# nilsbore/gp_compressor

Measured on AMD Instinct MI355X. Metric: patches/sec (compress+predict), higher is better.
Workload: dtype f64; 1 GPU; C2 room scan: 8192 patches x 256 pts per GPU, RBF + Gaussian noise, dense Cholesky fit + predictive mean on the 20x20 grid (m=400); patches_per_gpu=8192, points_per_patch=256, grid_points=400, parallelism=1 GPU, kernel=dense_mfma_w1

## Files before the change

gp_compressor_amd/csrc/dense_mfma_w1.hip:

```cpp
#include <cstdio>
#include <cstdlib>
#include <type_traits>

#include "gpc_device.h"
#include "dense_internal.h"
#include "mfma_tile.h"

#define W1_NPAD_MAX 512
#define W1_C 4
#define W1_NDT 10
#define W1_NT_OF(npad) ((npad) / 16)
#define W1_TRI_OF(npad) (W1_NT_OF(npad) * (W1_NT_OF(npad) + 1) / 2)
#define W1_TILE(i, j) (((size_t)(i) * (size_t)((i) + 1) / 2 + (size_t)(j)) * MF_IMG)


struct W1Params {
    DenseArgs a;
    double c_exp;
    double pivot_tol;
    double cs, noise_u, sfp, a_out;
    double* ws;
    double* linvt;
    int export_factor;
    unsigned long long* stamps;
};
#define W1_NPH 12
#ifdef W1_STAMPS
#define W1_STAMP(ph)                                                                                                 \
    do {                                                                                                             \
        __builtin_amdgcn_sched_barrier(0);                                                                           \
        const unsigned long long t_now_ = __builtin_amdgcn_s_memtime();                                              \
        st_acc_[ph] += t_now_ - t_prev_;                                                                             \
        t_prev_ = t_now_;                                                                                            \
        __builtin_amdgcn_sched_barrier(0);                                                                           \
    } while (0)
#else
#define W1_STAMP(ph) do { } while (0)
#endif

#define W1_LDS_SYNC()                                                                                                \
    do {                                                                                                             \
        __builtin_amdgcn_fence(__ATOMIC_SEQ_CST, "wavefront");                                                       \
        __builtin_amdgcn_wave_barrier();                                                                             \
    } while (0)

template <int A, int B, typename F>
__device__ static __forceinline__ void w1_static_for(F&& f)
{
    if constexpr (A < B) {
        f(std::integral_constant<int, A>{});
        w1_static_for<A + 1, B>(f);
    }
}
__host__ __device__ constexpr int w1_stream_col(int q)
{
    int kk = 0;
    while ((kk + 1) * (kk + 2) / 2 <= q) ++kk;
    return kk;
}
#define W1_BW 20

__device__ static __forceinline__ d4 w1_mfma4_neg(d4 a, d4 b, d4 acc)
{
#pragma unroll
    for (int s = 0; s < 4; ++s) acc = __builtin_amdgcn_mfma_f64_16x16x4f64(a[s], b[s], acc, 0, 0, 1);
    return acc;
}
__device__ static __forceinline__ d4 w1_trsm(d4 lv, d4 src)
{
    const d4 z4 = d4{0.0, 0.0, 0.0, 0.0};
    d4 D = __builtin_amdgcn_mfma_f64_16x16x4f64(lv[0], src[0], z4, 0, 0, 0);
    D = __builtin_amdgcn_mfma_f64_16x16x4f64(lv[1], src[1], D, 0, 0, 0);
    D = __builtin_amdgcn_mfma_f64_16x16x4f64(lv[2], src[2], D, 0, 0, 0);
    return __builtin_amdgcn_mfma_f64_16x16x4f64(lv[3], src[3], D, 0, 0, 0);
}

template <int MODE, int CNT, bool DIAG>
__device__ static __forceinline__ void w1_gram_row(d4 (&v)[W1_C], const double* px0, const double* px1, const double* T, double sf, bool scale_sf,
                                                   double cexp, double noise, bool dbl, int n, int r, int c0, int lr, int lg)
{
    const int pi = MF_TS * r + lr;
    const double xi0 = px0[pi], xi1 = px1[pi];
#pragma unroll
    for (int t = 0; t < CNT; ++t) {
#pragma unroll
        for (int q = 0; q < 4; ++q) {
            const int pj = MF_TS * (c0 + t) + lg + 4 * q;
            const double d0 = xi0 - px0[pj], d1 = xi1 - px1[pj];
            const double sq = __builtin_fma(d0, d0, d1 * d1);
            v[t][q] = MODE == 0 ? gpc_exp_neg(cexp * sq, T) : gpc_expm_poly<MODE == 1 ? 7 : 5>(sq);
        }
    }
    if (scale_sf) {
#pragma unroll
        for (int t = 0; t < CNT; ++t)
#pragma unroll
            for (int q = 0; q < 4; ++q) v[t][q] *= sf;
    }
    if constexpr (DIAG) {
#pragma unroll
        for (int q = 0; q < 4; ++q) {
            double d = v[CNT - 1][q] + noise;
            if (dbl) d += noise;
            v[CNT - 1][q] = (lr == lg + 4 * q) ? d : v[CNT - 1][q];
        }
    }
    if (MF_TS * (r + 1) > n || MF_TS * (c0 + CNT) > n) {
#pragma unroll
        for (int t = 0; t < CNT; ++t) {
#pragma unroll
            for (int q = 0; q < 4; ++q) {
                const int pj = MF_TS * (c0 + t) + lg + 4 * q;
                if (pi >= n || pj >= n) v[t][q] = (pi == pj) ? 1.0 : 0.0;
            }
        }
    }
}

template <int W1_NPAD>
__global__ __launch_bounds__(64, 2) void dense_w1_kernel(W1Params g)
{
    constexpr int W1_NT = W1_NT_OF(W1_NPAD), W1_TRI = W1_TRI_OF(W1_NPAD);
    __shared__ __attribute__((aligned(16))) double T[GPC_EXP_TABLE_SIZE];
    __shared__ __attribute__((aligned(16))) double px0[W1_NPAD], px1[W1_NPAD], zv[W1_NPAD];
    __shared__ __attribute__((aligned(16))) double rsbuf[32], wsc[32];
    __shared__ __attribute__((aligned(16))) double LinvC[W1_C * MF_IMG];

    const DenseArgs& A = g.a;
    int lane = threadIdx.x;
    int lr = lane & 15, lg = lane >> 4;
#define W1_FRESH_LANE()                                                                                              \
    do {                                                                                                             \
        lane = mf_opaque(lane);                                                                                      \
        lr = lane & 15;                                                                                              \
        lg = lane >> 4;                                                                                              \
    } while (0)
    const int m = A.m;
    const double sf = A.prm.sigmaf_sq, cexp = g.c_exp;
    const bool dbl = A.prm.ref_double_noise != 0;
    const int patch = blockIdx.x;
    double* Lt = g.ws + (size_t)patch * W1_TRI * MF_IMG;
    double* LinvTg = g.linvt + (size_t)patch * W1_NT * MF_IMG;

    gpc_exp_table_init(T);
    {
        const int o = __builtin_amdgcn_readfirstlane(A.off[patch]);
        const int n = __builtin_amdgcn_readfirstlane(A.off[patch + 1]) - o;
        double* fs = A.f_star + (size_t)patch * m;
        __syncthreads();
        if (n <= 0 || n > W1_NPAD) {
            for (int p = lane; p < m; p += 64) fs[p] = (n == 0) ? 0.0 : __builtin_nan("");
            if (lane == 0 && A.status) A.status[patch] = (n == 0) ? GPC_STATUS_OK : GPC_STATUS_NAN;
            return;
        }
        const int nt = __builtin_amdgcn_readfirstlane((n + MF_TS - 1) / MF_TS);
#ifdef W1_STAMPS
        unsigned long long st_acc_[W1_NPH] = {};
        unsigned long long t_prev_ = __builtin_amdgcn_s_memtime();
#endif

        const double xo0 = A.x0[o], xo1 = A.x1[o];
        double qr0[W1_NPAD / 64], qr1[W1_NPAD / 64];
        double mn0 = xo0, mx0 = xo0, mn1 = xo1, mx1 = xo1;
#pragma unroll
        for (int u = 0; u < W1_NPAD / 64; ++u) {
            const int i = lane + 64 * u;
            const bool live = i < n;
            qr0[u] = live ? A.x0[o + i] : xo0;
            qr1[u] = live ? A.x1[o + i] : xo1;
            mn0 = __builtin_fmin(mn0, qr0[u]); mx0 = __builtin_fmax(mx0, qr0[u]);
            mn1 = __builtin_fmin(mn1, qr1[u]); mx1 = __builtin_fmax(mx1, qr1[u]);
            zv[i] = live ? A.y[o + i] : 0.0;
        }
#pragma unroll
        for (int o_ = 32; o_ > 0; o_ >>= 1) {
            mn0 = __builtin_fmin(mn0, __shfl_xor(mn0, o_, 64)); mx0 = __builtin_fmax(mx0, __shfl_xor(mx0, o_, 64));
            mn1 = __builtin_fmin(mn1, __shfl_xor(mn1, o_, 64)); mx1 = __builtin_fmax(mx1, __shfl_xor(mx1, o_, 64));
        }
        int mode_g, mode_p;
        {
            const bool nan_box = !((mx0 - mn0) + (mx1 - mn1) < __builtin_inf());
            const double rx = mx0 - mn0, ry = mx1 - mn1;
            const double tg = nan_box ? __builtin_inf() : -cexp * __builtin_fma(rx, rx, ry * ry);
            const double hb = 0.5 * A.grid_res;
            const double bx = hb + __builtin_fmax(__builtin_fabs(mn0), __builtin_fabs(mx0));
            const double by = hb + __builtin_fmax(__builtin_fabs(mn1), __builtin_fabs(mx1));
            const double bq = __builtin_fmax(bx, by);
            const double tp = nan_box ? __builtin_inf() : -cexp * (bq * bq);
            mode_g = __builtin_amdgcn_readfirstlane(tg <= GPC_EXP_TINY_MAX ? 2 : tg <= GPC_EXP_SMALL_MAX ? 1 : 0);
            mode_p = __builtin_amdgcn_readfirstlane(tp <= GPC_EXP_TINY_MAX ? 2 : tp <= GPC_EXP_SMALL_MAX ? 1 : 0);
            if (mode_g == 0) mode_p = 0;
        }
        const bool scaled = mode_g > 0;
        {
            const double cs = scaled ? g.cs : 1.0;
            const double co0 = scaled ? xo0 : 0.0, co1 = scaled ? xo1 : 0.0;
#pragma unroll
            for (int u = 0; u < W1_NPAD / 64; ++u) {
                const int i = lane + 64 * u;
                const bool live = i < n;
                px0[i] = live ? cs * (qr0[u] - co0) : 0.0;
                px1[i] = live ? cs * (qr1[u] - co1) : 0.0;
            }
        }
        const bool scale_sf = g.export_factor != 0;
        const double noise_u = g.noise_u, ptol = g.pivot_tol;
        W1_LDS_SYNC();
#define W1_GRAM_ROW(v, CNT, DIAG, r, c0)                                                                              \
    do {                                                                                                             \
        if (mode_g == 2) w1_gram_row<2, CNT, DIAG>(v, px0, px1, T, sf, scale_sf, cexp, noise_u, dbl, n, r, c0, lr, lg);   \
        else if (mode_g == 1) w1_gram_row<1, CNT, DIAG>(v, px0, px1, T, sf, scale_sf, cexp, noise_u, dbl, n, r, c0, lr, lg); \
        else w1_gram_row<0, CNT, DIAG>(v, px0, px1, T, sf, scale_sf, cexp, noise_u, dbl, n, r, c0, lr, lg);            \
    } while (0)

        auto bw_step = [&](auto P, const d4 img, d4& pa) __attribute__((always_inline)) {
            constexpr int q = decltype(P)::value;
            constexpr int kk = w1_stream_col(q), t = q - kk * (kk + 1) / 2;
            if (kk < nt) {
                const int k = nt - 1 - kk;
                if constexpr (t < kk) {
                    const double a_ = zv[MF_TS * (k + 1 + t) + lr];
                    pa += img * a_;
                } else {
                    d4 ub = d4{0.0, 0.0, 0.0, 0.0};
                    if constexpr (kk > 0) {
                        const double tot = mf_row_reduce4(pa, lr);
                        if ((lr & 3) == 0) wsc[lg + 4 * (lr >> 2)] = tot;
                        W1_LDS_SYNC();
                        if (lr == 0) {
#pragma unroll
                            for (int q4 = 0; q4 < 4; ++q4) ub[q4] = zv[MF_TS * k + lg + 4 * q4] - wsc[lg + 4 * q4];
                        }
                    } else {
                        if (lr == 0) {
#pragma unroll
                            for (int q4 = 0; q4 < 4; ++q4) ub[q4] = zv[MF_TS * k + lg + 4 * q4];
                        }
                    }
                    const d4 al = w1_trsm(img, ub);
                    W1_LDS_SYNC();
                    if (lr == 0) {
#pragma unroll
                        for (int r = 0; r < 4; ++r) zv[MF_TS * k + lg + 4 * r] = al[r];
                    }
                    W1_LDS_SYNC();
                    pa = d4{0.0, 0.0, 0.0, 0.0};
                }
            }
        };
        bool bad = false;
        W1_STAMP(0);
#define W1_BLOCK_ROW(bi, kb, nb)                                                                                     \
    do {                                                                                                             \
        if ((bi) < (nb)) {                                                                                           \
            d4 gv[W1_C];                                                                                             \
            W1_GRAM_ROW(gv, (bi) + 1, true, (kb) + (bi), (kb));                                                      \
            _Pragma("unroll") for (int bc = 0; bc <= (bi); ++bc) tacc[(bi) * ((bi) + 1) / 2 + bc] = gv[bc];           \
        } else {                                                                                                     \
            _Pragma("unroll") for (int bc = 0; bc <= (bi); ++bc) tacc[(bi) * ((bi) + 1) / 2 + bc] = d4{0.0, 0.0, 0.0, 0.0}; \
        }                                                                                                            \
    } while (0)
#define W1_BLOCK_INIT(kb, nb)                                                                                        \
    do {                                                                                                             \
        _Pragma("unroll") for (int i = 0; i < W1_C; ++i) part[i] = 0.0;                                              \
                                             \
        __builtin_amdgcn_sched_barrier(0);                                                                           \
        W1_BLOCK_ROW(3, kb, nb);                                                                                     \
        __builtin_amdgcn_sched_barrier(0);                                                                           \
        W1_BLOCK_ROW(2, kb, nb);                                                                                     \
        __builtin_amdgcn_sched_barrier(0);                                                                           \
        W1_BLOCK_ROW(1, kb, nb);                                                                                     \
        __builtin_amdgcn_sched_barrier(0);                                                                           \
        W1_BLOCK_ROW(0, kb, nb);                                                                                     \
        __builtin_amdgcn_sched_barrier(0);                                                                           \
    } while (0)
        W1_STAMP(1);
        for (int k = 0;; k += W1_C) {
            const int nc = min(W1_C, nt - k);
            const int kl = k - 1;
            const bool last_step = k + W1_C >= nt;
            (void)last_step;
            W1_FRESH_LANE();
            const double* rrow[W1_C];
#pragma unroll
            for (int i = 0; i < W1_C; ++i) rrow[i] = Lt + W1_TILE(k + min(i, nc - 1), 0);
            d4 tacc[W1_NDT];
            double part[W1_C];
            d4 op[2][W1_C];
#pragma unroll
            for (int i = 0; i < W1_C; ++i) op[0][i] = op[1][i] = d4{0.0, 0.0, 0.0, 0.0};
            if (k > 0) {
#pragma unroll
                for (int i = 0; i < W1_C; ++i) op[0][i] = mf_img_load(rrow[i], lane);
            }
            W1_BLOCK_INIT(k, nc);
            for (int j = 0; j < k; j += 2) {
#pragma unroll
                for (int h = 0; h < 2; ++h) {
                    const int jn = min(j + h + 1, kl);
#pragma unroll
                    for (int i = 0; i < W1_C; ++i) op[h ^ 1][i] = mf_img_load(rrow[i] + (size_t)jn * MF_IMG, lane);
#pragma unroll
                    for (int d = 0; d < W1_NDT; ++d) {
                        const int bi = d >= 6 ? 3 : d >= 3 ? 2 : d >= 1 ? 1 : 0, bc = d - bi * (bi + 1) / 2;
                        if (bi < nc) tacc[d] = w1_mfma4_neg(op[h][bc], op[h][bi], tacc[d]);
                    }
                    const double* zq = zv + MF_TS * (j + h) + lg;
                    const double z0 = zq[0], z1 = zq[4], z2 = zq[8], z3 = zq[12];
#pragma unroll
                    for (int c = 0; c < W1_C; ++c) part[c] += (op[h][c][0] * z0 + op[h][c][1] * z1) + (op[h][c][2] * z2 + op[h][c][3] * z3);
                }
            }
            W1_STAMP(2);
            W1_FRESH_LANE();
            d4 Lb[W1_C * (W1_C - 1) / 2];
#pragma unroll
            for (int q = 0; q < W1_C * (W1_C - 1) / 2; ++q) Lb[q] = d4{0.0, 0.0, 0.0, 0.0};
            bool ok = mf_diag_factor_c(tacc[0], rsbuf, LinvC, LinvTg + (size_t)k * MF_IMG, ptol, lane);
            W1_LDS_SYNC();
            if (g.export_factor) mf_img_store(Lt + W1_TILE(k, k), lane, mf_img_load(LinvC, lane));
#pragma unroll
            for (int i = 1; i < W1_C; ++i) {
                if (ok && i < nc) {
#pragma unroll
                    for (int c = 0; c < i; ++c) {
                        d4 Tt = tacc[i * (i + 1) / 2 + c];
#pragma unroll
                        for (int c2 = 0; c2 < c; ++c2) Tt = w1_mfma4_neg(Lb[c * (c - 1) / 2 + c2], Lb[i * (i - 1) / 2 + c2], Tt);
                        const d4 lvc = mf_img_load(LinvC + c * MF_IMG, mf_opaque(lane));
                        const d4 L = w1_trsm(lvc, Tt);
                        Lb[i * (i - 1) / 2 + c] = L;
                        mf_img_store(Lt + W1_TILE(k + i, k + c), lane, L);
                    }
                    d4 Dii = tacc[i * (i + 1) / 2 + i];
#pragma unroll
                    for (int c = 0; c < i; ++c) Dii = w1_mfma4_neg(Lb[i * (i - 1) / 2 + c], Lb[i * (i - 1) / 2 + c], Dii);
                    ok = mf_diag_factor_c(Dii, rsbuf, LinvC + i * MF_IMG, LinvTg + (size_t)(k + i) * MF_IMG, ptol, lane);
                    W1_LDS_SYNC();
                    if (g.export_factor) mf_img_store(Lt + W1_TILE(k + i, k + i), lane, mf_img_load(LinvC + i * MF_IMG, mf_opaque(lane)));
                }
            }
            if (!ok) { bad = true; break; }
            W1_STAMP(3);
            W1_FRESH_LANE();
#pragma unroll
            for (int c = 0; c < W1_C; ++c) {
                if (c < nc) {
                    const int pj = MF_TS * (k + c) + lr;
                    double pp = part[c];
#pragma unroll
                    for (int c2 = 0; c2 < c; ++c2) {
                        const d4 lb = Lb[c * (c - 1) / 2 + c2];
                        const double* zq = zv + MF_TS * (k + c2) + lg;
                        pp += (lb[0] * zq[0] + lb[1] * zq[4]) + (lb[2] * zq[8] + lb[3] * zq[12]);
                    }
                    pp += __shfl_xor(pp, 16, 64);
                    pp += __shfl_xor(pp, 32, 64);
                    const double yv = zv[pj];
                    W1_LDS_SYNC();
                    if (lg == 0) zv[pj] = yv - pp;
                    W1_LDS_SYNC();
                    const d4 lv = mf_img_load(LinvC + c * MF_IMG, mf_opaque(lane));
                    const double* tq = zv + MF_TS * (k + c) + lg;
                    double zz = (lv[0] * tq[0] + lv[1] * tq[4]) + (lv[2] * tq[8] + lv[3] * tq[12]);
                    zz += __shfl_xor(zz, 16, 64);
                    zz += __shfl_xor(zz, 32, 64);
                    W1_LDS_SYNC();
                    if (lg == 0) zv[pj] = zz;
                    W1_LDS_SYNC();
                }
            }
            W1_STAMP(4);
            const int rows_tot = nt - (k + nc);
            if (rows_tot == 0) {
                __syncthreads();
                break;
            }
            if (k > 0) __syncthreads();
            const int npass = (rows_tot + 3) / 4;
            const int klp = k - 1;
            if (k == 0) {
                for (int pi_ = 0; pi_ < npass; ++pi_) {
                    const int first_row0 = (pi_ + 1 < npass) ? 4 * (pi_ + 1) : 0;
                    const int np4 = min(4, rows_tot - first_row0);
                    W1_FRESH_LANE();
                    d4 cy[W1_C][4];
#pragma unroll
                    for (int t = 0; t < 4; ++t) {
                        const int r_ = W1_C + first_row0 + min(t, np4 - 1);
                        d4 gv[W1_C];
                        W1_GRAM_ROW(gv, 2, false, r_, 0);
                        cy[0][t] = gv[0]; cy[1][t] = gv[1];
                        __builtin_amdgcn_sched_barrier(0);
                        W1_GRAM_ROW(gv, 2, false, r_, 2);
                        cy[2][t] = gv[0]; cy[3][t] = gv[1];
                        __builtin_amdgcn_sched_barrier(0);
                    }
                    W1_STAMP(5);
#pragma unroll
                    for (int c = 0; c < W1_C; ++c) {
                        const d4 lv = mf_img_load(LinvC + c * MF_IMG, mf_opaque(lane));
#pragma unroll
                        for (int t = 0; t < 4; ++t) {
#pragma unroll
                            for (int c2 = 0; c2 < c; ++c2) cy[c][t] = w1_mfma4_neg(Lb[c * (c - 1) / 2 + c2], cy[c2][t], cy[c][t]);
                            cy[c][t] = w1_trsm(lv, cy[c][t]);
                            if (t < np4) mf_img_store(Lt + W1_TILE(W1_C + first_row0 + t, c), lane, cy[c][t]);
                        }
                    }
                    W1_STAMP(7);
                }
            }
            if (k > 0) {
                for (int pi_ = 0; pi_ < npass; ++pi_) {
                    const int first_row = (pi_ + 1 < npass) ? 4 * (pi_ + 1) : 0;
                    const int np4 = min(4, rows_tot - first_row);
                    W1_FRESH_LANE();
                    d4 cy[W1_C][4];
                    int rr[4];
                    const double* rw_[4];
#pragma unroll
                    for (int t = 0; t < 4; ++t) {
                        rr[t] = k + W1_C + first_row + min(t, np4 - 1);
                        rw_[t] = Lt + W1_TILE(rr[t], 0);
                    }
                    d4 A2[2][W1_C], B[4];
#pragma unroll
                    for (int c = 0; c < W1_C; ++c) A2[0][c] = mf_img_load(rrow[c], lane);
#pragma unroll
                    for (int t = 0; t < 4; ++t) B[t] = mf_img_load(rw_[t], lane);
#pragma unroll
                    for (int t = 0; t < 4; ++t) {
                        d4 gv[W1_C];
                        W1_GRAM_ROW(gv, 2, false, rr[t], k);
                        cy[0][t] = gv[0]; cy[1][t] = gv[1];
                        __builtin_amdgcn_sched_barrier(0);
                        W1_GRAM_ROW(gv, 2, false, rr[t], k + 2);
                        cy[2][t] = gv[0]; cy[3][t] = gv[1];
                        __builtin_amdgcn_sched_barrier(0);
                    }
                    W1_STAMP(5);
                    d4 Lq[W1_C * (W1_C - 1) / 2];
#define W1_PASS_J(st, jn, PREFETCH)                                                                                  \
    do {                                                                                                             \
                                      \
        if (PREFETCH) {                                                                                              \
            _Pragma("unroll") for (int c = 0; c < W1_C; ++c) A2[(st) ^ 1][c] = mf_img_load(rrow[c] + (size_t)(jn) * MF_IMG, lane); \
        }                                                                                                            \
        __builtin_amdgcn_sched_barrier(0);                                                                           \
        _Pragma("unroll") for (int t = 0; t < 4; ++t) {                                                              \
            _Pragma("unroll") for (int c = 0; c < W1_C; ++c) cy[c][t] = w1_mfma4_neg(A2[st][c], B[t], cy[c][t]);      \
            __builtin_amdgcn_sched_barrier(0);                                                                       \
            if (PREFETCH) B[t] = mf_img_load(rw_[t] + (size_t)(jn) * MF_IMG, lane);                                    \
            else {      \
                if (t < 3) Lq[t] = mf_img_load(Lt + W1_TILE(k + (t == 0 ? 1 : 2), k + (t == 2 ? 1 : 0)), lane);      \
                else {                                                                                               \
                    _Pragma("unroll") for (int c2 = 0; c2 < 3; ++c2) Lq[3 + c2] = mf_img_load(Lt + W1_TILE(k + 3, k + c2), lane); \
                }                                                                                                    \
            }                                                                                                        \
            __builtin_amdgcn_sched_barrier(0);                                                                       \
        }                                                                                                            \
    } while (0)
                    for (int j = 0; j + 2 < k; j += 2) {
                        W1_PASS_J(0, j + 1, true);
                        W1_PASS_J(1, j + 2, true);
                    }
                    W1_PASS_J(0, klp, true);
                    W1_PASS_J(1, klp, false);
#undef W1_PASS_J
                    W1_STAMP(6);
                    W1_FRESH_LANE();
#pragma unroll
                    for (int c = 0; c < W1_C; ++c) {
                        const d4 lv = mf_img_load(LinvC + c * MF_IMG, mf_opaque(lane));
#pragma unroll
                        for (int t = 0; t < 4; ++t) {
#pragma unroll
                            for (int c2 = 0; c2 < c; ++c2) cy[c][t] = w1_mfma4_neg(Lq[c * (c - 1) / 2 + c2], cy[c2][t], cy[c][t]);
                            cy[c][t] = w1_trsm(lv, cy[c][t]);
                            if (t < np4) mf_img_store(Lt + W1_TILE(rr[t], k + c), lane, cy[c][t]);
                        }
                    }
                    W1_STAMP(7);
                }
            }
            __syncthreads();
            W1_STAMP(8);
        }
#undef W1_BLOCK_INIT
#undef W1_BLOCK_ROW

        if (bad) {
            for (int p = lane; p < m; p += 64) fs[p] = __builtin_nan("");
            if (A.alpha_out)
                for (int i = lane; i < n; i += 64) A.alpha_out[o + i] = __builtin_nan("");
            if (lane == 0 && A.status) A.status[patch] = GPC_STATUS_NOT_SPD;
            return;
        }

        {
            W1_FRESH_LANE();
            constexpr int NP = W1_NPAD / MF_TS;
            constexpr int SLEN = NP * (NP + 1) / 2;
            d4 win[W1_BW];
            auto stream_addr = [&](auto P) __attribute__((always_inline)) -> const double* {
                constexpr int q = decltype(P)::value;
                constexpr int kk = w1_stream_col(q), t = q - kk * (kk + 1) / 2;
                const int kq = max(nt - 1 - kk, 0);
                const double* ad = (t < kk) ? Lt + W1_TILE(kq + 1 + t, kq) : LinvTg + (size_t)kq * MF_IMG;
                return kk < nt ? ad : Lt;
            };
            w1_static_for<0, W1_BW>([&](auto P) __attribute__((always_inline)) {
                constexpr int q = decltype(P)::value;
                win[q] = mf_img_load_nt(stream_addr(P), lane);
            });
            d4 pa = d4{0.0, 0.0, 0.0, 0.0};
            w1_static_for<0, SLEN>([&](auto P) __attribute__((always_inline)) {
                constexpr int q = decltype(P)::value;
                bw_step(P, win[q % W1_BW], pa);
                if constexpr (q + W1_BW < SLEN) {
                    win[q % W1_BW] = mf_img_load_nt(stream_addr(std::integral_constant<int, q + W1_BW>{}), lane);
                }
            });
        }
        W1_STAMP(9);
        double* av = zv;
        if (A.alpha_out)
            for (int i = lane; i < n; i += 64) A.alpha_out[o + i] = av[i] * g.a_out;

        W1_FRESH_LANE();
        if (m <= 0) {
        } else if (A.xs0 == nullptr && A.grid_sz <= 32) {
            const int sz = A.grid_sz;
            const double res = A.grid_res;
            d4 P[2][2];
#pragma unroll
            for (int mt = 0; mt < 2; ++mt)
#pragma unroll
                for (int nl = 0; nl < 2; ++nl) P[mt][nl] = d4{0.0, 0.0, 0.0, 0.0};
            double gqx[2], gqy[2];
            const double cs = scaled ? g.cs : 1.0, co0 = scaled ? A.x0[o] : 0.0, co1 = scaled ? A.x1[o] : 0.0;
            const double argc = scaled ? -1.0 : cexp, sfp = g.sfp;
#pragma unroll
            for (int h = 0; h < 2; ++h) {
                const double gq = res * (((double)(16 * h + lr) + 0.5) / (double)sz - 0.5);
                gqx[h] = cs * (gq - co0);
                gqy[h] = cs * (gq - co1);
            }
            auto predict_loop = [&](auto mode_tag) __attribute__((always_inline)) {
                constexpr int MP = decltype(mode_tag)::value;
                for (int ibase = 0; ibase < n; ibase += 32) {
#pragma unroll
                    for (int s = 0; s < 8; ++s) {
                        const int i = ibase + 4 * s + lg;
                        const int ic = min(i, W1_NPAD - 1);
                        const double al = (i < n) ? sfp * av[ic] : 0.0;
                        const double xi0 = px0[ic], xi1 = px1[ic];
                        double ea[2], eb[2];
#pragma unroll
                        for (int h = 0; h < 2; ++h) {
                            const double dy = gqy[h] - xi1, dx = gqx[h] - xi0;
                            if constexpr (MP == 0) {
                                ea[h] = gpc_exp_neg(argc * (dy * dy), T);
                                eb[h] = gpc_exp_neg(argc * (dx * dx), T) * al;
                            } else {
                                ea[h] = gpc_expm_poly<MP == 1 ? 7 : 5>(dy * dy);
                                eb[h] = gpc_expm_poly<MP == 1 ? 7 : 5>(dx * dx) * al;
                            }
                        }
#pragma unroll
                        for (int nl = 0; nl < 2; ++nl)
#pragma unroll
                            for (int mt = 0; mt < 2; ++mt)
                                P[mt][nl] = __builtin_amdgcn_mfma_f64_16x16x4f64(ea[mt], eb[nl], P[mt][nl], 0, 0, 0);
                    }
                }
            };
            if (mode_p == 2) predict_loop(std::integral_constant<int, 2>{});
            else if (mode_p == 1) predict_loop(std::integral_constant<int, 1>{});
            else predict_loop(std::integral_constant<int, 0>{});
#pragma unroll
            for (int mt = 0; mt < 2; ++mt)
#pragma unroll
                for (int nl = 0; nl < 2; ++nl)
#pragma unroll
                    for (int r = 0; r < 4; ++r) {
                        const int py = 16 * mt + lg + 4 * r, pxx = 16 * nl + lr;
                        if (py < sz && pxx < sz) fs[py * sz + pxx] = P[mt][nl][r];
                    }
        } else {
            const double cs = scaled ? g.cs : 1.0, co0 = scaled ? A.x0[o] : 0.0, co1 = scaled ? A.x1[o] : 0.0;
            const double argc = scaled ? -1.0 : cexp, sfp = g.sfp;
            for (int p = lane; p < m; p += 64) {
                double q0, q1;
                if (A.xs0) {
                    q0 = A.xs0[p];
                    q1 = A.xs1[p];
                } else {
                    const int gx = p % A.grid_sz, gy = p / A.grid_sz;
                    q0 = A.grid_res * (((double)gx + 0.5) / (double)A.grid_sz - 0.5);
                    q1 = A.grid_res * (((double)gy + 0.5) / (double)A.grid_sz - 0.5);
                }
                q0 = cs * (q0 - co0);
                q1 = cs * (q1 - co1);
                double s_ = 0.0;
                for (int i = 0; i < n; ++i) {
                    const double d0 = px0[i] - q0, d1 = px1[i] - q1;
                    s_ += gpc_exp_neg(argc * __builtin_fma(d0, d0, d1 * d1), T) * av[i];
                }
                fs[p] = sfp * s_;
            }
        }
        if (lane == 0 && A.status) A.status[patch] = GPC_STATUS_OK;
#ifdef W1_STAMPS
        W1_STAMP(10);
        if (g.stamps && lane == 0)
            for (int q_ = 0; q_ < W1_NPH; ++q_) atomicAdd(g.stamps + q_, st_acc_[q_]);
#endif
    }
}

static int w1_npad(const DenseArgs& a) { return a.n_max <= 256 ? 256 : W1_NPAD_MAX; }

bool dense_w1_supported(const DenseArgs& a)
{
    if (a.v_star) return a.n_max <= 256 && a.ny == 1 && !a.sel && a.xs0 != nullptr;
    return a.n_max <= W1_NPAD_MAX && a.ny == 1 && !a.sel;
}

#define W1_MAX_SLOTS 8192
static int w1_chunk(const DenseArgs& a, int cap_in)
{
    const char* e = getenv("GPC_W1_SLOTS");
    int cap = e && atoi(e) > 0 ? atoi(e) : W1_MAX_SLOTS;
    if (cap_in > 0 && cap_in < cap) cap = cap_in;
    return a.P < cap ? a.P : cap;
}

size_t dense_w1_ws_bytes(const gpc_ctx* ctx, const DenseArgs& a, int* grid_out, int cap)
{
    (void)ctx;
    const int grid = w1_chunk(a, cap);
    if (grid_out) *grid_out = grid;
    const int npad = w1_npad(a);
    return sizeof(double) * ((size_t)(W1_TRI_OF(npad) + W1_NT_OF(npad)) * MF_IMG * (size_t)grid + (a.v_star ? (size_t)a.n_total : 0));
}

int dense_w1_launch(gpc_ctx* ctx, const DenseSite& site, const DenseArgs& a_in, int grid)
{
    DenseArgs a = a_in;
    double* v_star = a.v_star;
    a.v_star = nullptr;
    W1Params g;
    g.c_exp = (double)(-0.5f) / a.prm.l_sq;
    g.ws = reinterpret_cast<double*>(dense_ws(ctx, site));
    const int npad = w1_npad(a);
    g.linvt = g.ws + (size_t)W1_TRI_OF(npad) * MF_IMG * (size_t)grid;
    g.export_factor = v_star ? 1 : 0;
    const double sf = a.prm.sigmaf_sq;
    const bool unit = !v_star;
    g.cs = sqrt(-g.c_exp);
    g.noise_u = unit ? a.prm.noise / sf : a.prm.noise;
    g.pivot_tol = GPC_PIVOT_RTOL * (unit ? 1.0 + a.prm.noise / sf : sf + a.prm.noise);
    g.sfp = unit ? 1.0 : sf;
    g.a_out = unit ? 1.0 / sf : 1.0;
    g.stamps = nullptr;
    if (v_star) {
        a.m = 0;
        if (!a.alpha_out) a.alpha_out = g.linvt + (size_t)W1_NT_OF(npad) * MF_IMG * (size_t)grid;
    }
    ctx->last_dense_kernel = v_star ? "dense_mfma_w1 + dense_variance" : npad == 256 ? "dense_mfma_w1" : "dense_mfma_w1_512";
#ifdef W1_STAMPS
    if (getenv("GPC_W1_STAMPS")) {
        GPC_HIP(ctx, hipMalloc(&g.stamps, sizeof(unsigned long long) * W1_NPH));
        GPC_HIP(ctx, hipMemsetAsync(g.stamps, 0, sizeof(unsigned long long) * W1_NPH, site.stream));
    }
#endif
    for (int base = 0; base < a.P; base += grid) {
        const int cnt = a.P - base < grid ? a.P - base : grid;
        g.a = a;
        g.a.P = cnt;
        g.a.off = a.off + base;
        g.a.f_star = a.f_star ? a.f_star + (size_t)base * a.ny * a_in.m : nullptr;
        g.a.status = a.status ? a.status + base : nullptr;
        if (npad == 256) hipLaunchKernelGGL((dense_w1_kernel<256>), dim3(cnt), dim3(64), 0, site.stream, g);
        else hipLaunchKernelGGL((dense_w1_kernel<W1_NPAD_MAX>), dim3(cnt), dim3(64), 0, site.stream, g);
        GPC_HIP(ctx, hipGetLastError());
        if (v_star) {
            DenseArgs av = g.a;
            av.m = a_in.m;
            const int rc = dense_variance_launch(ctx, site, av, W1_NT_OF(256), g.ws, a.alpha_out, v_star + (size_t)base * a_in.m);
            if (rc != GPC_OK) return rc;
        }
    }
#ifdef W1_STAMPS
    if (g.stamps) {
        unsigned long long h[W1_NPH];
        GPC_HIP(ctx, hipStreamSynchronize(site.stream));
        GPC_HIP(ctx, hipMemcpy(h, g.stamps, sizeof(h), hipMemcpyDeviceToHost));
        (void)hipFree(g.stamps);
        static const char* names[W1_NPH] = {"load", "sweep gram", "sweep loop", "chain", "forward", "pass gram", "pass loop", "pass trsm",
                                            "step fence", "backward", "predict", ""};
        unsigned long long tot = 0;
        for (int q = 0; q < W1_NPH; ++q) tot += h[q];
        fprintf(stderr, "[GPC_W1_STAMPS] mean s_memtime ticks per patch (total %.0f)\n", (double)tot / a.P);
        for (int q = 0; q < 11; ++q) fprintf(stderr, "  %-12s %9.0f  %5.1f %%\n", names[q], (double)h[q] / a.P, 100.0 * h[q] / tot);
    }
#endif
    return GPC_OK;
}
```

Measured before the change: 5.494 million patches/s.

## Carry next diagonal block's Schur update from panel tail into the next step

For the NPAD=256 specialization, the last panel pass of each blocked Cholesky step now runs an eager tail. That tail computes the next diagonal block's trailing update (tacc) and the z-partial sums (cpart) straight from the freshly solved panel tiles in registers. The next step then starts its Gram accumulation from the carried values and skips the last W1_C columns of the left-looking j-loop, which avoids reloading those tiles from memory. The cost is more register pressure from tacc and cpart living across iterations, plus a more complex ordering of passes where the first-row pass moves to the end.

```diff
diff --git a/gp_compressor_amd/csrc/dense_mfma_w1.hip b/gp_compressor_amd/csrc/dense_mfma_w1.hip
--- a/gp_compressor_amd/csrc/dense_mfma_w1.hip
+++ b/gp_compressor_amd/csrc/dense_mfma_w1.hip
@@ -121,6 +121,7 @@
 __global__ __launch_bounds__(64, 2) void dense_w1_kernel(W1Params g)
 {
     constexpr int W1_NT = W1_NT_OF(W1_NPAD), W1_TRI = W1_TRI_OF(W1_NPAD);
+    constexpr bool CARRY = W1_NPAD == 256;
     __shared__ __attribute__((aligned(16))) double T[GPC_EXP_TABLE_SIZE];
     __shared__ __attribute__((aligned(16))) double px0[W1_NPAD], px1[W1_NPAD], zv[W1_NPAD];
     __shared__ __attribute__((aligned(16))) double rsbuf[32], wsc[32];
@@ -255,8 +256,9 @@
         if ((bi) < (nb)) {                                                                                           \
             d4 gv[W1_C];                                                                                             \
             W1_GRAM_ROW(gv, (bi) + 1, true, (kb) + (bi), (kb));                                                      \
-            _Pragma("unroll") for (int bc = 0; bc <= (bi); ++bc) tacc[(bi) * ((bi) + 1) / 2 + bc] = gv[bc];           \
-        } else {                                                                                                     \
+            _Pragma("unroll") for (int bc = 0; bc <= (bi); ++bc)                                                     \
+                tacc[(bi) * ((bi) + 1) / 2 + bc] = CARRY ? tacc[(bi) * ((bi) + 1) / 2 + bc] + gv[bc] : gv[bc];       \
+        } else if (!CARRY) {    \
             _Pragma("unroll") for (int bc = 0; bc <= (bi); ++bc) tacc[(bi) * ((bi) + 1) / 2 + bc] = d4{0.0, 0.0, 0.0, 0.0}; \
         }                                                                                                            \
     } while (0)
@@ -275,26 +277,31 @@
         __builtin_amdgcn_sched_barrier(0);                                                                           \
     } while (0)
         W1_STAMP(1);
+        d4 tacc[W1_NDT];
+        double cpart[W1_C];
+#pragma unroll
+        for (int d = 0; d < W1_NDT; ++d) tacc[d] = d4{0.0, 0.0, 0.0, 0.0};
+#pragma unroll
+        for (int i = 0; i < W1_C; ++i) cpart[i] = 0.0;
         for (int k = 0;; k += W1_C) {
             const int nc = min(W1_C, nt - k);
-            const int kl = k - 1;
+            const int ks = CARRY ? k - W1_C : k, kl = ks - 1;
             const bool last_step = k + W1_C >= nt;
             (void)last_step;
             W1_FRESH_LANE();
             const double* rrow[W1_C];
 #pragma unroll
             for (int i = 0; i < W1_C; ++i) rrow[i] = Lt + W1_TILE(k + min(i, nc - 1), 0);
-            d4 tacc[W1_NDT];
             double part[W1_C];
             d4 op[2][W1_C];
 #pragma unroll
             for (int i = 0; i < W1_C; ++i) op[0][i] = op[1][i] = d4{0.0, 0.0, 0.0, 0.0};
-            if (k > 0) {
+            if (ks > 0) {
 #pragma unroll
                 for (int i = 0; i < W1_C; ++i) op[0][i] = mf_img_load(rrow[i], lane);
             }
             W1_BLOCK_INIT(k, nc);
-            for (int j = 0; j < k; j += 2) {
+            for (int j = 0; j < ks; j += 2) {
 #pragma unroll
                 for (int h = 0; h < 2; ++h) {
                     const int jn = min(j + h + 1, kl);
@@ -310,6 +317,10 @@
 #pragma unroll
                     for (int c = 0; c < W1_C; ++c) part[c] += (op[h][c][0] * z0 + op[h][c][1] * z1) + (op[h][c][2] * z2 + op[h][c][3] * z3);
                 }
+            }
+            if constexpr (CARRY) {
+#pragma unroll
+                for (int c = 0; c < W1_C; ++c) part[c] += cpart[c];
             }
             W1_STAMP(2);
             W1_FRESH_LANE();
@@ -376,26 +387,65 @@
                 __syncthreads();
                 break;
             }
-            if (k > 0) __syncthreads();
+            if (CARRY || k > 0) __syncthreads();
             const int npass = (rows_tot + 3) / 4;
             const int klp = k - 1;
+#define W1_EAGER_TAIL()                                                                                              \
+    do {                                                                                                             \
+        _Pragma("unroll") for (int c = 0; c < W1_C; ++c) {                                                           \
+            const d4 lv = mf_img_load(LinvC + c * MF_IMG, mf_opaque(lane));                                          \
+            _Pragma("unroll") for (int t = 0; t < 4; ++t) {                                                          \
+                cy[c][t] = w1_trsm(lv, cy[c][t]);                                                                    \
+                if (t < np4) mf_img_store(Lt + W1_TILE(k + W1_C + t, k + c), lane, cy[c][t]);                        \
+            }                                                                                                        \
+            __builtin_amdgcn_sched_barrier(0);                                                                       \
+            _Pragma("unroll") for (int c3 = c + 1; c3 < W1_C; ++c3) {                                                \
+                _Pragma("unroll") for (int t = 0; t < 4; ++t)                                                        \
+                    cy[c3][t] = w1_mfma4_neg(Lq[c3 * (c3 - 1) / 2 + c], cy[c][t], cy[c3][t]);                        \
+            }                                                                                                        \
+            __builtin_amdgcn_sched_barrier(0);                                                                       \
+            {                                                                                                        \
+                const double* zq = zv + MF_TS * (k + c) + lg;                                                        \
+                const double z0 = zq[0], z1 = zq[4], z2 = zq[8], z3 = zq[12];                                        \
+                _Pragma("unroll") for (int i = 0; i < W1_C; ++i) {                                                   \
+                    const double pz = (cy[c][i][0] * z0 + cy[c][i][1] * z1) + (cy[c][i][2] * z2 + cy[c][i][3] * z3); \
+                    cpart[i] = c == 0 ? pz : cpart[i] + pz;                                                          \
+                    asm volatile("" : "+v"(cpart[i]));    \
+                }                                                                                                    \
+            }                                                                                                        \
+            _Pragma("unroll") for (int bc = 0; bc < W1_C; ++bc) {                                                    \
+                _Pragma("unroll") for (int bi = bc; bi < W1_C; ++bi) {                                               \
+                    const int d = bi * (bi + 1) / 2 + bc;                                                            \
+                    tacc[d] = w1_mfma4_neg(cy[c][bc], cy[c][bi], c == 0 ? d4{0.0, 0.0, 0.0, 0.0} : tacc[d]);         \
+                }                                                                                                    \
+            }                                                                                                        \
+            _Pragma("unroll") for (int c3 = c + 2; c3 < W1_C; ++c3)                                                  \
+                Lq[c3 * (c3 - 1) / 2 + c + 1] = mf_img_load(Lt + W1_TILE(k + c3, k + c + 1), mf_opaque(lane));       \
+            __builtin_amdgcn_sched_barrier(0);                                                                       \
+        }                                                                                                            \
+    } while (0)
+#define W1_PASS_GRAM()                                                                                               \
+    do {                                                                                                             \
+        _Pragma("unroll") for (int t = 0; t < 4; ++t) {                                                              \
+            d4 gv[W1_C];                                                                                             \
+            W1_GRAM_ROW(gv, 2, false, rr[t], k);                                                                     \
+            cy[0][t] = gv[0]; cy[1][t] = gv[1];                                                                      \
+            __builtin_amdgcn_sched_barrier(0);                                                                       \
+            W1_GRAM_ROW(gv, 2, false, rr[t], k + 2);                                                                 \
+            cy[2][t] = gv[0]; cy[3][t] = gv[1];                                                                      \
+            __builtin_amdgcn_sched_barrier(0);                                                                       \
+        }                                                                                                            \
+    } while (0)
             if (k == 0) {
-                for (int pi_ = 0; pi_ < npass; ++pi_) {
-                    const int first_row0 = (pi_ + 1 < npass) ? 4 * (pi_ + 1) : 0;
+                for (int pi_ = 0; pi_ + (CARRY ? 1 : 0) < npass; ++pi_) {
+                    const int first_row0 = (CARRY || pi_ + 1 < npass) ? 4 * (pi_ + 1) : 0;
                     const int np4 = min(4, rows_tot - first_row0);
                     W1_FRESH_LANE();
                     d4 cy[W1_C][4];
-#pragma unroll
-                    for (int t = 0; t < 4; ++t) {
-                        const int r_ = W1_C + first_row0 + min(t, np4 - 1);
-                        d4 gv[W1_C];
-                        W1_GRAM_ROW(gv, 2, false, r_, 0);
-                        cy[0][t] = gv[0]; cy[1][t] = gv[1];
-                        __builtin_amdgcn_sched_barrier(0);
-                        W1_GRAM_ROW(gv, 2, false, r_, 2);
-                        cy[2][t] = gv[0]; cy[3][t] = gv[1];
-                        __builtin_amdgcn_sched_barrier(0);
-                    }
+                    int rr[4];
+#pragma unroll
+                    for (int t = 0; t < 4; ++t) rr[t] = W1_C + first_row0 + min(t, np4 - 1);
+                    W1_PASS_GRAM();
                     W1_STAMP(5);
 #pragma unroll
                     for (int c = 0; c < W1_C; ++c) {
@@ -410,38 +460,43 @@
                     }
                     W1_STAMP(7);
                 }
-            }
-            if (k > 0) {
-                for (int pi_ = 0; pi_ < npass; ++pi_) {
-                    const int first_row = (pi_ + 1 < npass) ? 4 * (pi_ + 1) : 0;
-                    const int np4 = min(4, rows_tot - first_row);
+                if constexpr (CARRY) {
+                    const int np4 = min(4, rows_tot);
                     W1_FRESH_LANE();
                     d4 cy[W1_C][4];
                     int rr[4];
-                    const double* rw_[4];
-#pragma unroll
-                    for (int t = 0; t < 4; ++t) {
-                        rr[t] = k + W1_C + first_row + min(t, np4 - 1);
-                        rw_[t] = Lt + W1_TILE(rr[t], 0);
-                    }
-                    d4 A2[2][W1_C], B[4];
-#pragma unroll
-                    for (int c = 0; c < W1_C; ++c) A2[0][c] = mf_img_load(rrow[c], lane);
-#pragma unroll
-                    for (int t = 0; t < 4; ++t) B[t] = mf_img_load(rw_[t], lane);
-#pragma unroll
-                    for (int t = 0; t < 4; ++t) {
-                        d4 gv[W1_C];
-                        W1_GRAM_ROW(gv, 2, false, rr[t], k);
-                        cy[0][t] = gv[0]; cy[1][t] = gv[1];
-                        __builtin_amdgcn_sched_barrier(0);
-                        W1_GRAM_ROW(gv, 2, false, rr[t], k + 2);
-                        cy[2][t] = gv[0]; cy[3][t] = gv[1];
-                        __builtin_amdgcn_sched_barrier(0);
-                    }
+#pragma unroll
+                    for (int t = 0; t < 4; ++t) rr[t] = W1_C + min(t, np4 - 1);
+                    d4 Lq[W1_C * (W1_C - 1) / 2];
+#pragma unroll
+                    for (int t = 0; t < 3; ++t) Lq[t == 2 ? 3 : t] = mf_img_load(Lt + W1_TILE(1 + t, 0), lane);
+                    W1_PASS_GRAM();
                     W1_STAMP(5);
-                    d4 Lq[W1_C * (W1_C - 1) / 2];
-#define W1_PASS_J(st, jn, PREFETCH)                                                                                  \
+                    W1_FRESH_LANE();
+                    W1_EAGER_TAIL();
+                    W1_STAMP(7);
+                }
+            }
+            int k_later = k;
+            if constexpr (CARRY) asm volatile("" : "+s"(k_later));
+            if (k_later > 0) {
+#define W1_PASS_HEAD(first_row)                                                                                      \
+    const int np4 = min(4, rows_tot - (first_row));                                                                  \
+    W1_FRESH_LANE();                                                                                                 \
+    d4 cy[W1_C][4];                                                                  \
+    int rr[4];                                                                                                       \
+    const double* rw_[4];                                                                                            \
+    _Pragma("unroll") for (int t = 0; t < 4; ++t) {                                                                  \
+        rr[t] = k + W1_C + (first_row) + min(t, np4 - 1);         \
+        rw_[t] = Lt + W1_TILE(rr[t], 0);                                                                             \
+    }                                                                                                                \
+    d4 A2[2][W1_C], B[4];                                                                                            \
+    _Pragma("unroll") for (int c = 0; c < W1_C; ++c) A2[0][c] = mf_img_load(rrow[c], lane);                          \
+    _Pragma("unroll") for (int t = 0; t < 4; ++t) B[t] = mf_img_load(rw_[t], lane);                                  \
+    W1_PASS_GRAM();                                                                                                  \
+    W1_STAMP(5);                                                                                                     \
+    d4 Lq[W1_C * (W1_C - 1) / 2];
+#define W1_PASS_J(st, jn, PREFETCH, ALLQ)                                                                            \
     do {                                                                                                             \
                                       \
         if (PREFETCH) {                                                                                              \
@@ -452,22 +507,29 @@
             _Pragma("unroll") for (int c = 0; c < W1_C; ++c) cy[c][t] = w1_mfma4_neg(A2[st][c], B[t], cy[c][t]);      \
             __builtin_amdgcn_sched_barrier(0);                                                                       \
             if (PREFETCH) B[t] = mf_img_load(rw_[t] + (size_t)(jn) * MF_IMG, lane);                                    \
-            else {      \
+            else if (ALLQ) {      \
                 if (t < 3) Lq[t] = mf_img_load(Lt + W1_TILE(k + (t == 0 ? 1 : 2), k + (t == 2 ? 1 : 0)), lane);      \
                 else {                                                                                               \
                     _Pragma("unroll") for (int c2 = 0; c2 < 3; ++c2) Lq[3 + c2] = mf_img_load(Lt + W1_TILE(k + 3, k + c2), lane); \
                 }                                                                                                    \
+            } else {                                                                                                 \
+                if (t < 3) Lq[t == 2 ? 3 : t] = mf_img_load(Lt + W1_TILE(k + 1 + t, k), lane);                       \
             }                                                                                                        \
             __builtin_amdgcn_sched_barrier(0);                                                                       \
         }                                                                                                            \
     } while (0)
-                    for (int j = 0; j + 2 < k; j += 2) {
-                        W1_PASS_J(0, j + 1, true);
-                        W1_PASS_J(1, j + 2, true);
-                    }
-                    W1_PASS_J(0, klp, true);
-                    W1_PASS_J(1, klp, false);
-#undef W1_PASS_J
+#define W1_PASS_LOOP(ALLQ)                                                                                           \
+    do {                                                                                                             \
+        for (int j = 0; j + 2 < k; j += 2) {                                                                         \
+            W1_PASS_J(0, j + 1, true, ALLQ);                                                                         \
+            W1_PASS_J(1, j + 2, true, ALLQ);                                                                         \
+        }                                                                                                            \
+        W1_PASS_J(0, klp, true, ALLQ);                 \
+        W1_PASS_J(1, klp, false, ALLQ);                                                                              \
+    } while (0)
+                for (int pi_ = 0; pi_ + (CARRY ? 1 : 0) < npass; ++pi_) {
+                    W1_PASS_HEAD((CARRY || pi_ + 1 < npass) ? 4 * (pi_ + 1) : 0)
+                    W1_PASS_LOOP(true);
                     W1_STAMP(6);
                     W1_FRESH_LANE();
 #pragma unroll
@@ -483,7 +545,21 @@
                     }
                     W1_STAMP(7);
                 }
-            }
+                if constexpr (CARRY) {
+                    W1_PASS_HEAD(0)
+                    W1_PASS_LOOP(false);
+                    W1_STAMP(6);
+                    W1_FRESH_LANE();
+                    W1_EAGER_TAIL();
+                    W1_STAMP(7);
+                }
+#undef W1_PASS_LOOP
+#undef W1_PASS_J
+#undef W1_PASS_HEAD
+            }
+#undef W1_PASS_GRAM
+#undef W1_EAGER_TAIL
+            if constexpr (CARRY) W1_FRESH_LANE();
             __syncthreads();
             W1_STAMP(8);
         }
```

After: 5.447 million patches/s. No clear change (-0.9%).
